# zju3dv/RelightableAvatar

Measured on AMD Instinct MI355X. Metric: rays_per_sec, higher is better.
Workload: dtype f16

## Files before the change

relightableavatar_amd/csrc/ra_hdq.hip:

```cpp
#include "ra_kernels.hpp"
#include <type_traits>
#include <cstdlib>

namespace {

constexpr int KNN_THREADS = 256;

#ifdef RA_COARSE_TS
__device__ long long ra_coarse_ts[64 * 64 * 16 * 8];
extern "C" int ra_coarse_read_timestamps(long long* out) { return (int)hipMemcpyFromSymbol(out, HIP_SYMBOL(ra_coarse_ts), sizeof(ra_coarse_ts)); }
#define RA_CSTAMP(k) do { if (tsp) { __builtin_amdgcn_sched_barrier(0); if ((threadIdx.x & 63) == 0) tsp[k] = __builtin_readcyclecounter(); __builtin_amdgcn_sched_barrier(0); } } while (0)
#else
#define RA_CSTAMP(k) do { } while (0)
#endif
constexpr int VT = 2048;

__device__ __forceinline__ void inv3d(const float R[9], float M[9]) {
    M[0] = R[4] * R[8] - R[7] * R[5];
    M[3] = -R[3] * R[8] + R[6] * R[5];
    M[6] = R[3] * R[7] - R[6] * R[4];
    M[1] = -R[1] * R[8] + R[7] * R[2];
    M[4] = R[0] * R[8] - R[6] * R[2];
    M[7] = -R[0] * R[7] + R[6] * R[1];
    M[2] = R[1] * R[5] - R[4] * R[2];
    M[5] = -R[0] * R[5] + R[3] * R[2];
    M[8] = R[0] * R[4] - R[3] * R[1];
    const float D = R[0] * M[0] + R[1] * M[3] + R[2] * M[6];
    const float inv = 1.f / (D + 1e-8f);
#pragma unroll
    for (int i = 0; i < 9; ++i) M[i] *= inv;
}

__device__ __forceinline__ float sgn(float x) { return (x > 0.f) ? 1.f : ((x < 0.f) ? -1.f : 0.f); }

__global__ void vert_blend_kernel(const float* __restrict__ weights, const float* __restrict__ A, const float* __restrict__ big_A,
                                  int n_verts, int n_bones, float* __restrict__ vertA) {
    const int v = blockIdx.x * blockDim.x + threadIdx.x;
    if (v >= n_verts) return;
    float acc[24];
#pragma unroll
    for (int e = 0; e < 24; ++e) acc[e] = 0.f;
    for (int j = 0; j < n_bones; ++j) {
        const float w = weights[(size_t)v * n_bones + j];
#pragma unroll
        for (int e = 0; e < 12; ++e) {
            acc[e] += w * A[j * 16 + e];
            acc[12 + e] += w * big_A[j * 16 + e];
        }
    }
#pragma unroll
    for (int e = 0; e < 24; ++e) vertA[(size_t)v * 24 + e] = acc[e];
}

__global__ void pack_verts_kernel(const float* __restrict__ pv, int n, float4* __restrict__ out) {
    const int v = blockIdx.x * blockDim.x + threadIdx.x;
    if (v < n) out[v] = make_float4(pv[3 * v], pv[3 * v + 1], pv[3 * v + 2], 0.f);
}

__global__ __launch_bounds__(256) void fold_bias_kernel(const float* __restrict__ W, int ld, int col0, int ncond, const float* __restrict__ cond,
                                                        const float* __restrict__ bias, float* __restrict__ out) {
    const int r = blockIdx.x * 4 + (threadIdx.x >> 6), lane = threadIdx.x & 63;
    if (r >= 256) return;
    const float* row = W + (size_t)r * ld + col0;
    float a = 0.f;
    for (int c = lane; c < ncond; c += 64) a = fmaf(row[c], cond[c], a);
#pragma unroll
    for (int o = 32; o > 0; o >>= 1) a += __shfl_xor(a, o);
    if (lane == 0) out[r] = bias[r] + a;
}

constexpr int BVH_THREADS = 1024;
constexpr int BVH_LEAF = 32;
constexpr int BVH_FAN = 8;
constexpr int BVH_MAXN = 16384;
constexpr int BVH_MAXL = BVH_MAXN / BVH_LEAF;
constexpr int BVH_MAXS = BVH_MAXL / BVH_FAN;

__device__ __forceinline__ unsigned expand10(unsigned v) {
    v = (v * 0x00010001u) & 0xFF0000FFu;
    v = (v * 0x00000101u) & 0x0F00F00Fu;
    v = (v * 0x00000011u) & 0xC30C30C3u;
    v = (v * 0x00000005u) & 0x49249249u;
    return v;
}

constexpr int RANK_WAVES = BVH_THREADS / 64;

__global__ __launch_bounds__(BVH_THREADS) void bvh_rank_kernel(const float4* __restrict__ pv, int n, int* __restrict__ order) {
    __shared__ unsigned long long keys[BVH_MAXN];
    __shared__ float red[6][BVH_THREADS / 64];
    __shared__ float bb[6];
    __shared__ int cnt[RANK_WAVES][64];
    const int tid = threadIdx.x;
    float mn[3] = {3e38f, 3e38f, 3e38f}, mx[3] = {-3e38f, -3e38f, -3e38f};
    for (int i = tid; i < n; i += BVH_THREADS) {
        const float4 v = pv[i];
        mn[0] = fminf(mn[0], v.x); mn[1] = fminf(mn[1], v.y); mn[2] = fminf(mn[2], v.z);
        mx[0] = fmaxf(mx[0], v.x); mx[1] = fmaxf(mx[1], v.y); mx[2] = fmaxf(mx[2], v.z);
    }
#pragma unroll
    for (int c = 0; c < 3; ++c)
#pragma unroll
        for (int o = 32; o > 0; o >>= 1) { mn[c] = fminf(mn[c], __shfl_xor(mn[c], o)); mx[c] = fmaxf(mx[c], __shfl_xor(mx[c], o)); }
    if ((tid & 63) == 0) for (int c = 0; c < 3; ++c) { red[c][tid >> 6] = mn[c]; red[3 + c][tid >> 6] = mx[c]; }
    __syncthreads();
    if (tid < 6) {
        float a = red[tid][0];
        for (int w = 1; w < BVH_THREADS / 64; ++w) a = tid < 3 ? fminf(a, red[tid][w]) : fmaxf(a, red[tid][w]);
        bb[tid] = a;
    }
    __syncthreads();
    const int n4 = (n + 3) & ~3;
    for (int i = tid; i < n4; i += BVH_THREADS) {
        unsigned long long k = ~0ull;
        if (i < n) {
            const float4 v = pv[i];
            const float p[3] = {v.x, v.y, v.z};
            unsigned q[3];
#pragma unroll
            for (int c = 0; c < 3; ++c) {
                const float e = fmaxf(bb[3 + c] - bb[c], 1e-12f);
                q[c] = (unsigned)fminf(fmaxf((p[c] - bb[c]) / e * 1023.f, 0.f), 1023.f);
            }
            const unsigned code = (expand10(q[0]) << 2) | (expand10(q[1]) << 1) | expand10(q[2]);
            k = ((unsigned long long)code << 32) | (unsigned)i;
        }
        keys[i] = k;
    }
    __syncthreads();
    const int lane = tid & 63, g = tid >> 6;
    const int e = blockIdx.x * 64 + lane;
    const unsigned long long mine = e < n ? keys[e] : 0ull;
    const int chunk = ((n4 / 4 + RANK_WAVES - 1) / RANK_WAVES) * 4;
    const int j0 = g * chunk, j1 = min(n4, j0 + chunk);
    int c = 0;
    for (int j = j0; j < j1; j += 4) {
        const ulonglong2 a = *reinterpret_cast<const ulonglong2*>(&keys[j]);
        const ulonglong2 b = *reinterpret_cast<const ulonglong2*>(&keys[j + 2]);
        c += (a.x < mine) + (a.y < mine) + (b.x < mine) + (b.y < mine);
    }
    cnt[g][lane] = c;
    __syncthreads();
    if (g == 0 && e < n) {
        int r = 0;
#pragma unroll
        for (int w = 0; w < RANK_WAVES; ++w) r += cnt[w][lane];
        order[r] = e;
    }
}

__global__ __launch_bounds__(BVH_THREADS) void bvh_boxes_kernel(const float4* __restrict__ pv, const int* __restrict__ order, int n,
                                                                float* __restrict__ leaves, float4* __restrict__ sbox, int nl, int ns) {
    __shared__ float lb[BVH_MAXL][6];
    const int tid = threadIdx.x, e = tid & 31;
    for (int l = tid >> 5; l < nl; l += BVH_THREADS / 32) {
        const int i = l * BVH_LEAF + e;
        float4 v = make_float4(__int_as_float(0x7f800000), __int_as_float(0x7f800000), __int_as_float(0x7f800000), __int_as_float(0x7fffffff));
        float lo[3] = {3e38f, 3e38f, 3e38f}, hi[3] = {-3e38f, -3e38f, -3e38f};
        if (i < n) {
            const int id = order[i];
            v = pv[id];
            v.w = __int_as_float(id);
            lo[0] = hi[0] = v.x; lo[1] = hi[1] = v.y; lo[2] = hi[2] = v.z;
        }
        float* soa = leaves + (size_t)l * (4 * BVH_LEAF) + e;
        soa[0] = v.x; soa[BVH_LEAF] = v.y; soa[2 * BVH_LEAF] = v.z; soa[3 * BVH_LEAF] = v.w;
#pragma unroll
        for (int c = 0; c < 3; ++c)
#pragma unroll
            for (int o = 16; o > 0; o >>= 1) { lo[c] = fminf(lo[c], __shfl_xor(lo[c], o)); hi[c] = fmaxf(hi[c], __shfl_xor(hi[c], o)); }
        if (e == 0) {
#pragma unroll
            for (int c = 0; c < 3; ++c) { lb[l][c] = lo[c]; lb[l][3 + c] = hi[c]; }
        }
    }
    __syncthreads();
    for (int sidx = tid; sidx < ns; sidx += BVH_THREADS) {
        float lo[3] = {3e38f, 3e38f, 3e38f}, hi[3] = {-3e38f, -3e38f, -3e38f};
        for (int k = 0; k < BVH_FAN; ++k) {
            const int l = sidx * BVH_FAN + k;
            if (l < nl)
#pragma unroll
                for (int c = 0; c < 3; ++c) { lo[c] = fminf(lo[c], lb[l][c]); hi[c] = fmaxf(hi[c], lb[l][3 + c]); }
        }
        sbox[2 * sidx] = make_float4(lo[0], lo[1], lo[2], 0.f);
        sbox[2 * sidx + 1] = make_float4(hi[0], hi[1], hi[2], 0.f);
        float* rec = reinterpret_cast<float*>(sbox + 2 * (size_t)ns) + (size_t)sidx * (6 * BVH_FAN);
        for (int k = 0; k < BVH_FAN; ++k) {
            const int l = sidx * BVH_FAN + k;
#pragma unroll
            for (int c = 0; c < 6; ++c) rec[12 * (k >> 1) + 2 * c + (k & 1)] = l < nl ? lb[l][c] : (c < 3 ? 3e38f : -3e38f);
        }
    }
}

template <int I, int N, typename F>
__device__ __forceinline__ void static_for(F&& f) {
    if constexpr (I < N) {
        f(std::integral_constant<int, I>{});
        static_for<I + 1, N>(f);
    }
}

template <int K>
__device__ __forceinline__ float row_bcast(float v) {
    return __int_as_float(__builtin_amdgcn_update_dpp(0, __float_as_int(v), 0x150 + K, 0xf, 0xf, false));
}

__device__ __forceinline__ float box_dist2(const float p[3], float lx, float ly, float lz, float hx, float hy, float hz) {
    const float dx = fmaxf(fmaxf(lx - p[0], p[0] - hx), 0.f);
    const float dy = fmaxf(fmaxf(ly - p[1], p[1] - hy), 0.f);
    const float dz = fmaxf(fmaxf(lz - p[2], p[2] - hz), 0.f);
    return dx * dx + dy * dy + dz * dz;
}

__device__ __forceinline__ float dist2(float dx, float dy, float dz) { return __fmaf_rn(dz, dz, __fmaf_rn(dx, dx, dy * dy)); }

__device__ __forceinline__ void knn_insert(float d, int id, float& d0, float& d1, float& d2, int& i0, int& i1, int& i2, bool dedup = false) {
    if (__builtin_expect(__ballot(d <= d2) == 0ull, 1)) return;
    bool fresh = true;
    if (dedup) fresh = (id != i0) & (id != i1) & (id != i2);
    const bool c2 = fresh && (d < d2 || (d == d2 && id < i2));
    const bool c1 = fresh && (d < d1 || (d == d1 && id < i1));
    const bool c0 = fresh && (d < d0 || (d == d0 && id < i0));
    const float nd2 = c1 ? d1 : (c2 ? d : d2);
    const int ni2 = c1 ? i1 : (c2 ? id : i2);
    const float nd1 = c0 ? d0 : (c1 ? d : d1);
    const int ni1 = c0 ? i0 : (c1 ? id : i1);
    d0 = c0 ? d : d0;
    i0 = c0 ? id : i0;
    d1 = nd1; i1 = ni1; d2 = nd2; i2 = ni2;
}

__device__ __forceinline__ void ray_point(const RaySet& rs, int i, float x[3]) {
    if (rs.mode == 0) {
        x[0] = rs.x[3 * i]; x[1] = rs.x[3 * i + 1]; x[2] = rs.x[3 * i + 2];
    } else if (rs.mode == 1) {
        const float t = rs.t[i];
        x[0] = rs.o[3 * i] + t * rs.d[3 * i];
        x[1] = rs.o[3 * i + 1] + t * rs.d[3 * i + 1];
        x[2] = rs.o[3 * i + 2] + t * rs.d[3 * i + 2];
    } else {
        const float t = rs.t[i];
        const int p = rs.pix[i], l = rs.light[i];
        x[0] = rs.o[3 * p] + t * rs.ldir[3 * l];
        x[1] = rs.o[3 * p + 1] + t * rs.ldir[3 * l + 1];
        x[2] = rs.o[3 * p + 2] + t * rs.ldir[3 * l + 2];
    }
}

template <bool BVH, int SPLIT, bool HINT = false>
__global__ __launch_bounds__(SPLIT == 1 ? KNN_THREADS : 64 * SPLIT) void hdq_coarse_kernel(FrameState fr, RaySet rs, int n_launch, float th, float inv2r2,
                                                                  HdqOut out, int dbg) {
    static_assert(SPLIT == 1 || (BVH && SPLIT >= 2 && SPLIT <= 16), "SPLIT > 1: the workgroup is SPLIT waves on the same 64 queries");
    constexpr int NT = SPLIT == 1 ? KNN_THREADS : 64 * SPLIT;
    __shared__ __attribute__((aligned(16))) unsigned char smem[BVH ? 16 : VT * 16];
#ifdef RA_COARSE_TS
    long long* tsp = blockIdx.x < 64 ? ra_coarse_ts + ((((dbg >> 8) & 63) * 64 + blockIdx.x) * 16 + (threadIdx.x >> 6)) * 8 : nullptr;
    dbg &= 255;
    if (tsp && (threadIdx.x & 63) == 0) { tsp[1] = tsp[2] = tsp[3] = tsp[4] = tsp[5] = tsp[6] = tsp[7] = 0; }
    RA_CSTAMP(0);
#endif
    const int n = rs.n_dev ? min(*rs.n_dev, n_launch) : n_launch;
    const int base = blockIdx.x * (SPLIT == 1 ? KNN_THREADS : 64);
    if (base >= n) return;
    if (blockIdx.x == 0 && threadIdx.x == 0 && out.counters) atomicAdd(&out.counters->n_coarse, (unsigned long long)n);
    const int i = base + (SPLIT == 1 ? threadIdx.x : (threadIdx.x & 63));
    const bool live_q = i < n && !(rs.skip && rs.skip[i < n ? i : 0]);
    bool live = live_q;
    if (__syncthreads_count(live_q) == 0) return;
    float x[3] = {0.f, 0.f, 0.f};
    if (live) ray_point(rs, i, x);
    const float xt[3] = {x[0] - fr.Th[0], x[1] - fr.Th[1], x[2] - fr.Th[2]};
    float p[3];
#pragma unroll
    for (int c = 0; c < 3; ++c) p[c] = xt[0] * fr.R[c] + xt[1] * fr.R[3 + c] + xt[2] * fr.R[6 + c];

    RA_CSTAMP(1);
    float d0 = 3.0e38f, d1 = 3.0e38f, d2 = 3.0e38f;
    int i0 = 0, i1 = 0, i2 = 0;
    if (dbg & 1) { d0 = 1e-4f; d1 = 2e-4f; d2 = 3e-4f; i0 = 0; i1 = 1; i2 = 2; }
    else if (BVH) {
        const int nl = fr.bvh_leaves, ns = fr.bvh_supers;
        if (!live) { d0 = d1 = d2 = -1.f; }
        const unsigned long long lm = __ballot(live);
        const int first = lm ? __ffsll((long long)lm) - 1 : 0;
        const int lane = threadIdx.x & 63;
        typedef float f2 __attribute__((ext_vector_type(2)));
        const f2 px2 = {p[0], p[0]}, py2 = {p[1], p[1]}, pz2 = {p[2], p[2]};
        constexpr bool hinted = HINT;
#ifdef RA_COARSE_TS
        int n_rare = 0;
#endif
        typedef float f8 __attribute__((ext_vector_type(8)));
        typedef float f4 __attribute__((ext_vector_type(4)));
        typedef int i4 __attribute__((ext_vector_type(4)));
        auto soa8 = [&](int off) __attribute__((always_inline)) { return *(const f8 __attribute__((address_space(4)))*)(fr.bvh_soa + off); };
        auto soa_id4 = [&](int off) __attribute__((always_inline)) { return *(const i4 __attribute__((address_space(4)))*)(fr.bvh_soa + off); };
        auto box4 = [&](int off) __attribute__((always_inline)) {
            return *(const f4 __attribute__((address_space(4)))*)(reinterpret_cast<const float*>(fr.bvh_sbox) + off);
        };
        auto box1 = [&](int off) __attribute__((always_inline)) { return reinterpret_cast<const float*>(fr.bvh_sbox)[off]; };
        auto scan_leaf = [&](int l) __attribute__((always_inline)) {
            const int L = l * (4 * BVH_LEAF);
            f8 cx = soa8(L), cy = soa8(L + BVH_LEAF), cz = soa8(L + 2 * BVH_LEAF), nx = cx, ny = cy, nz = cz;
            static_for<0, 4>([&](auto q_) {
                constexpr int q = decltype(q_)::value;
                static_for<0, 2>([&](auto g_) {
                    constexpr int g = decltype(g_)::value;
                    const f2 ax = {cx[4 * g], cx[4 * g + 1]}, ay = {cy[4 * g], cy[4 * g + 1]}, az = {cz[4 * g], cz[4 * g + 1]};
                    const f2 bx = {cx[4 * g + 2], cx[4 * g + 3]}, by = {cy[4 * g + 2], cy[4 * g + 3]}, bz = {cz[4 * g + 2], cz[4 * g + 3]};
                    const f2 dxa = px2 - ax, dya = py2 - ay, dza = pz2 - az, dxb = px2 - bx, dyb = py2 - by, dzb = pz2 - bz;
                    f2 da = dya * dya, db = dyb * dyb;
                    da = __builtin_elementwise_fma(dxa, dxa, da);
                    db = __builtin_elementwise_fma(dxb, dxb, db);
                    da = __builtin_elementwise_fma(dza, dza, da);
                    db = __builtin_elementwise_fma(dzb, dzb, db);
                    if (__builtin_expect(__ballot(fminf(fminf(da.x, da.y), fminf(db.x, db.y)) <= d2) != 0ull, 0)) {
#ifdef RA_COARSE_TS
                        ++n_rare;
#endif
                        const i4 id = soa_id4(L + 3 * BVH_LEAF + 8 * q + 4 * g);
                        knn_insert(da.x, id.x, d0, d1, d2, i0, i1, i2, hinted);
                        knn_insert(da.y, id.y, d0, d1, d2, i0, i1, i2, hinted);
                        knn_insert(db.x, id.z, d0, d1, d2, i0, i1, i2, hinted);
                        knn_insert(db.y, id.w, d0, d1, d2, i0, i1, i2, hinted);
                    }
                    if constexpr (g == 0 && q < 3) { nx = soa8(L + 8 * (q + 1)); ny = soa8(L + BVH_LEAF + 8 * (q + 1)); nz = soa8(L + 2 * BVH_LEAF + 8 * (q + 1)); }
                });
                cx = nx; cy = ny; cz = nz;
            });
        };
        int n_scan = 0, n_open = 0;
        if (lm != 0ull) {
            int seed = -1;
            if (hinted) {
                if (live) {
                    float e[3]; int h[3];
#pragma unroll
                    for (int k = 0; k < 3; ++k) {
                        h[k] = rs.hint_src ? rs.hint_src[3 * (size_t)rs.hint_src_index[i] + k] : rs.nn_hint[3 * (size_t)i + k];
                        const float4 v = fr.pverts4[h[k]];
                        e[k] = dist2(p[0] - v.x, p[1] - v.y, p[2] - v.z);
                    }
                    auto before = [&](int a, int b) { return e[a] < e[b] || (e[a] == e[b] && h[a] < h[b]); };
                    auto swap = [&](int a, int b) { const float te = e[a]; e[a] = e[b]; e[b] = te; const int th_ = h[a]; h[a] = h[b]; h[b] = th_; };
                    if (before(1, 0)) swap(0, 1);
                    if (before(2, 1)) swap(1, 2);
                    if (before(1, 0)) swap(0, 1);
                    d0 = e[0]; d1 = e[1]; d2 = e[2]; i0 = h[0]; i1 = h[1]; i2 = h[2];
                }
            } else {
                auto bc = [&](float v) __attribute__((always_inline)) { return __int_as_float(__builtin_amdgcn_readlane(__float_as_int(v), first)); };
                const float q[3] = {bc(p[0]), bc(p[1]), bc(p[2])};
                auto wave_argmin = [&](float d) __attribute__((always_inline)) {
                    float m = d;
#pragma unroll
                    for (int o = 32; o > 0; o >>= 1) m = fminf(m, __shfl_xor(m, o));
                    return __ffsll((long long)__ballot(d == m)) - 1;
                };
                float d = 3.4e38f;
                if (lane < ns) { const int o = 8 * lane; d = box_dist2(q, box1(o), box1(o + 1), box1(o + 2), box1(o + 4), box1(o + 5), box1(o + 6)); }
                const int bi = wave_argmin(d);
                d = 3.4e38f;
                if (lane < BVH_FAN) { const int o = 8 * ns + bi * (6 * BVH_FAN) + 12 * (lane >> 1) + (lane & 1); d = box_dist2(q, box1(o), box1(o + 2), box1(o + 4), box1(o + 6), box1(o + 8), box1(o + 10)); }
                seed = bi * BVH_FAN + wave_argmin(d);
            }
            RA_CSTAMP(2);
            if (!hinted) {
                n_scan = 1;
                scan_leaf(seed);
            }
            RA_CSTAMP(3);
#pragma unroll 1
            for (int j = SPLIT > 1 ? (int)(threadIdx.x >> 6) : 0; j < ns; j += SPLIT) {
                const f4 slo = box4(8 * j), shi = box4(8 * j + 4);
                if (__ballot(box_dist2(p, slo.x, slo.y, slo.z, shi.x, shi.y, shi.z) * 0.99999f <= d2) == 0ull) continue;
                ++n_open;
#pragma unroll 1
                for (int pr = 0; pr < BVH_FAN / 2; ++pr) {
                    const int ro = 8 * ns + j * (6 * BVH_FAN) + 12 * pr;
                    const f4 ra = box4(ro), rb = box4(ro + 4), rc = box4(ro + 8);
                    const f2 ax = f2{ra.x, ra.y} - px2, ay = f2{ra.z, ra.w} - py2, az = f2{rb.x, rb.y} - pz2;
                    const f2 bx = px2 - f2{rb.z, rb.w}, by = py2 - f2{rc.x, rc.y}, bz = pz2 - f2{rc.z, rc.w};
                    const f2 ex = {__builtin_fmaxf(__builtin_fmaxf(ax.x, bx.x), 0.f), __builtin_fmaxf(__builtin_fmaxf(ax.y, bx.y), 0.f)};
                    const f2 ey = {__builtin_fmaxf(__builtin_fmaxf(ay.x, by.x), 0.f), __builtin_fmaxf(__builtin_fmaxf(ay.y, by.y), 0.f)};
                    const f2 ez = {__builtin_fmaxf(__builtin_fmaxf(az.x, bz.x), 0.f), __builtin_fmaxf(__builtin_fmaxf(az.y, bz.y), 0.f)};
                    f2 dd = ex * ex;
                    dd = __builtin_elementwise_fma(ey, ey, dd);
                    dd = __builtin_elementwise_fma(ez, ez, dd);
                    dd *= 0.99999f;
                    const int l = j * BVH_FAN + 2 * pr;
                    if (l != seed && __ballot(dd.x <= d2) != 0ull) { scan_leaf(l); ++n_scan; }
                    if (l + 1 != seed && __ballot(dd.y <= d2) != 0ull) { scan_leaf(l + 1); ++n_scan; }
                }
            }
        }
        RA_CSTAMP(4);
#ifdef RA_COARSE_TS
        if (tsp && (threadIdx.x & 63) == 0) tsp[7] = ((long long)n_scan << 32) | ((long long)n_rare << 12) | n_open;
#endif
        if (SPLIT > 1) {
            __shared__ float md[SPLIT > 1 ? SPLIT - 1 : 1][3][64];
            __shared__ int mi[SPLIT > 1 ? SPLIT - 1 : 1][3][64];
            const int wv = threadIdx.x >> 6;
            if (wv > 0) {
                md[wv - 1][0][lane] = d0; md[wv - 1][1][lane] = d1; md[wv - 1][2][lane] = d2;
                mi[wv - 1][0][lane] = i0; mi[wv - 1][1][lane] = i1; mi[wv - 1][2][lane] = i2;
            }
            __syncthreads();
            if (wv == 0) {
#pragma unroll
                for (int w = 0; w < SPLIT - 1; ++w)
#pragma unroll
                    for (int k = 0; k < 3; ++k) {
                        const int id = mi[w][k][lane];
                        const bool dup = id == i0 || id == i1 || id == i2;
                        knn_insert(dup ? 3.4e38f : md[w][k][lane], id, d0, d1, d2, i0, i1, i2);
                    }
            } else {
                live = false;
            }
        }
        RA_CSTAMP(5);
        if ((dbg & 4) && out.counters && lane == 0) {
            atomicAdd(&out.counters->n_shadow_rays, (unsigned long long)n_scan);
            atomicAdd(&out.counters->n_hit_pixels, (unsigned long long)n_open);
        }
    } else {
        float4* sv = reinterpret_cast<float4*>(smem);
        for (int v0 = 0; v0 < fr.n_verts; v0 += VT) {
            const int nv = min(VT, fr.n_verts - v0);
            __syncthreads();
            for (int j = threadIdx.x; j < nv; j += KNN_THREADS) sv[j] = fr.pverts4[v0 + j];
            __syncthreads();
#pragma unroll 4
            for (int j = 0; j < nv; ++j) {
                const float4 v = sv[j];
                const float dx = p[0] - v.x, dy = p[1] - v.y, dz = p[2] - v.z;
                const float d = dist2(dx, dy, dz);
                knn_insert(d, v0 + j, d0, d1, d2, i0, i1, i2);
            }
        }
    }
    if (rs.nn_hint && live) {
        int* hw = rs.nn_hint + 3 * (size_t)i;
        hw[0] = i0; hw[1] = i1; hw[2] = i2;
    }
    if (dbg & 2) { if (live) out.sdf[i] = d0 + d1 + d2 + (float)(i0 + i1 + i2); return; }
    float dk[3] = {d0, d1, d2};
    int ik[3] = {i0, i1, i2};
    float sk[3];
#pragma unroll
    for (int k = 0; k < 3; ++k) {
        const float4 v = fr.pverts4[ik[k]];
        const float* nn = fr.pnorm + 3 * (size_t)ik[k];
        const float dot = (p[0] - v.x) * nn[0] + (p[1] - v.y) * nn[1] + (p[2] - v.z) * nn[2];
        sk[k] = sqrtf(dk[k]) * sgn(dot);
    }
    const float th2 = th * th;
    if (!(dbg & 32)) {
        const float* t0 = fr.tverts + 3 * (size_t)ik[0];
#pragma unroll
        for (int k = 1; k < 3; ++k) {
            const float* tk = fr.tverts + 3 * (size_t)ik[k];
            const float ex = tk[0] - t0[0], ey = tk[1] - t0[1], ez = tk[2] - t0[2];
            if (!(ex * ex + ey * ey + ez * ez < th2)) { dk[k] = dk[0]; ik[k] = ik[0]; sk[k] = sk[0]; }
        }
    }
    float smpl = (sk[0] + sk[1] + sk[2]) / 3.f;
    if (dbg & 32) {
        const float sg = fmaxf(fmaxf(sgn(sk[0]), sgn(sk[1])), sgn(sk[2]));
        smpl = sqrtf((dk[0] + dk[1] + dk[2]) / 3.f) * sg;
        sk[0] = sk[1] = sk[2] = smpl;
    }
    smpl = (smpl < -th) ? smpl : fabsf(smpl);
    const bool fine = live && (d0 < th2);
    if (live) {
        out.sdf[i] = smpl;
        if (out.raw_zero && !fine) {
            float* rz = out.raw_zero + (size_t)i * out.raw_C;
            for (int c = 0; c < out.raw_C; ++c) rz[c] = 0.f;
        }
        if (out.dbg_sdf_batch) {
#pragma unroll
            for (int k = 0; k < 3; ++k) { out.dbg_sdf_batch[3 * i + k] = sk[k]; out.dbg_nn_batch[3 * i + k] = ik[k]; out.dbg_d2[3 * i + k] = dk[k]; }
        }
    }
    __shared__ int wcount[NT / 64 + 1], wcount2[NT / 64 + 1];
    const bool fine2 = fine && out.key != nullptr && out.key[rs.light[i]] != 0;
    const unsigned long long m = __ballot(fine && !fine2), m2 = out.key ? __ballot(fine2) : 0ull;
    const int lane = threadIdx.x & 63, wv = threadIdx.x >> 6;
    if (lane == 0) { wcount[wv] = __popcll(m); wcount2[wv] = __popcll(m2); }
    __syncthreads();
    if (threadIdx.x == 0) {
        int tot = 0, tot2 = 0;
#pragma unroll
        for (int w = 0; w < NT / 64; ++w) { const int cnt = wcount[w]; wcount[w] = tot; tot += cnt; const int c2 = wcount2[w]; wcount2[w] = tot2; tot2 += c2; }
        wcount[NT / 64] = (dbg & 8) ? base : (tot ? atomicAdd(out.fine_count, tot) : 0);
        wcount2[NT / 64] = tot2 ? atomicAdd(out.fine_count2, tot2) : 0;
    }
    __syncthreads();
    RA_CSTAMP(6);
    if (!fine || (dbg & 16)) return;
    const int slot = fine2 ? wcount2[NT / 64] + wcount2[wv] + __popcll(m2 & ((1ull << lane) - 1ull))
                           : wcount[NT / 64] + wcount[wv] + __popcll(m & ((1ull << lane) - 1ull));
    float w[3], ws = 0.f;
#pragma unroll
    for (int k = 0; k < 3; ++k) { w[k] = expf(-dk[k] * inv2r2); ws += w[k]; }
    ws += 1.1920928955078125e-07f;
    float M[24];
#pragma unroll
    for (int e = 0; e < 24; ++e) M[e] = 0.f;
#pragma unroll
    for (int k = 0; k < 3; ++k) {
        const float wk = w[k] / ws;
        const float4* src = reinterpret_cast<const float4*>(fr.vertA + (size_t)ik[k] * 24);
#pragma unroll
        for (int q = 0; q < 6; ++q) {
            const float4 a = src[q];
            M[4 * q] += wk * a.x; M[4 * q + 1] += wk * a.y; M[4 * q + 2] += wk * a.z; M[4 * q + 3] += wk * a.w;
        }
    }
    const float AR[9] = {M[0], M[1], M[2], M[4], M[5], M[6], M[8], M[9], M[10]};
    float Ai[9];
    inv3d(AR, Ai);
    const float q[3] = {p[0] - M[3], p[1] - M[7], p[2] - M[11]};
    float tp[3], bp[3];
#pragma unroll
    for (int r = 0; r < 3; ++r) tp[r] = Ai[3 * r] * q[0] + Ai[3 * r + 1] * q[1] + Ai[3 * r + 2] * q[2];
#pragma unroll
    for (int r = 0; r < 3; ++r) bp[r] = M[12 + 4 * r] * tp[0] + M[12 + 4 * r + 1] * tp[1] + M[12 + 4 * r + 2] * tp[2] + M[12 + 4 * r + 3];
    if (fine2) {
        out.fine_idx2[slot] = i;
        out.bpts2[3 * slot] = bp[0]; out.bpts2[3 * slot + 1] = bp[1]; out.bpts2[3 * slot + 2] = bp[2];
        return;
    }
    out.fine_idx[slot] = i;
    out.bpts[3 * slot] = bp[0]; out.bpts[3 * slot + 1] = bp[1]; out.bpts[3 * slot + 2] = bp[2];
    if (out.mats) {
        float4* dst = reinterpret_cast<float4*>(out.mats + (size_t)slot * 24);
#pragma unroll
        for (int qd = 0; qd < 6; ++qd) dst[qd] = make_float4(M[4 * qd], M[4 * qd + 1], M[4 * qd + 2], M[4 * qd + 3]);
    }
    if (out.dbg_bpts) {
#pragma unroll
        for (int c = 0; c < 3; ++c) { out.dbg_bpts[3 * i + c] = bp[c]; out.dbg_tpts[3 * i + c] = tp[c]; }
#pragma unroll
        for (int e = 0; e < 24; ++e) out.dbg_mats[(size_t)i * 24 + e] = M[e];
    }
}

}

void launch_vert_blend(const float* weights, const float* A, const float* big_A, int n_verts, int n_bones, float* vertA,
                       hipStream_t s) {
    hipLaunchKernelGGL(vert_blend_kernel, dim3((n_verts + 255) / 256), dim3(256), 0, s, weights, A, big_A, n_verts, n_bones, vertA);
}

void launch_pack_verts(const float* pverts, int n_verts, float4* out, hipStream_t s) {
    hipLaunchKernelGGL(pack_verts_kernel, dim3((n_verts + 255) / 256), dim3(256), 0, s, pverts, n_verts, out);
}

void launch_fold_bias(const float* W, int ld, int col0, int ncond, const float* cond, const float* bias, float* out,
                      hipStream_t s) {
    hipLaunchKernelGGL(fold_bias_kernel, dim3(64), dim3(256), 0, s, W, ld, col0, ncond, cond, bias, out);
}

int bvh_leaf_count(int n_verts) {
    if (n_verts > BVH_MAXN) return 0;
    return (n_verts + BVH_LEAF - 1) / BVH_LEAF;
}
int bvh_super_count(int n_leaves) { return (n_leaves + BVH_FAN - 1) / BVH_FAN; }

void launch_bvh_build(const float4* pverts4, int n_verts, int* order, float* leaves, float4* sbox, int n_leaves, int n_supers, hipStream_t s) {
    hipLaunchKernelGGL(bvh_rank_kernel, dim3((n_verts + 63) / 64), dim3(BVH_THREADS), 0, s, pverts4, n_verts, order);
    hipLaunchKernelGGL(bvh_boxes_kernel, dim3(1), dim3(BVH_THREADS), 0, s, pverts4, order, n_verts, leaves, sbox, n_leaves, n_supers);
}

void launch_hdq_coarse(const FrameState& fr, const RaySet& rs, int n, float th, float blend_radius, const HdqOut& out,
                       hipStream_t s, bool geodesic) {
    if (n <= 0) return;
    const float inv2r2 = 1.f / (2.f * blend_radius * blend_radius);
    const dim3 grid((n + KNN_THREADS - 1) / KNN_THREADS);
    int dbg = 0, probe = 0, split_max = 196608;
#ifdef RA_TESTING
    static const int e_dbg = getenv("RA_COARSE_DBG") ? atoi(getenv("RA_COARSE_DBG")) : 0;
    static const int e_probe = getenv("RA_COARSE_PROBE") ? atoi(getenv("RA_COARSE_PROBE")) : 0;
    static const int e_split = getenv("RA_COARSE_SPLIT_MAX") ? atoi(getenv("RA_COARSE_SPLIT_MAX")) : 196608;
    dbg = e_dbg; probe = e_probe; split_max = e_split;
#endif
    if (!geodesic) dbg |= 32;
#ifdef RA_COARSE_TS
    static int launch_no = 0;
    dbg |= (launch_no++ & 63) << 8;
#endif
    const bool hint = (rs.nn_hint != nullptr && rs.hint_valid != 0) || rs.hint_src != nullptr;
    for (int pass = probe ? 0 : 1; pass < 2; ++pass) {
        const int d = pass == 0 ? probe : dbg;
        if (fr.bvh_leaves > 0 && n <= split_max)
        {
            const int groups = (n + 63) / 64;
            if (hint) {
                if (n <= split_max / 8) hipLaunchKernelGGL((hdq_coarse_kernel<true, 16, true>), dim3(groups), dim3(1024), 0, s, fr, rs, n, th, inv2r2, out, d);
                else if (n <= split_max / 2) hipLaunchKernelGGL((hdq_coarse_kernel<true, 8, true>), dim3(groups), dim3(512), 0, s, fr, rs, n, th, inv2r2, out, d);
                else hipLaunchKernelGGL((hdq_coarse_kernel<true, 4, true>), dim3(groups), dim3(256), 0, s, fr, rs, n, th, inv2r2, out, d);
            } else {
                if (n <= split_max / 8) hipLaunchKernelGGL((hdq_coarse_kernel<true, 16>), dim3(groups), dim3(1024), 0, s, fr, rs, n, th, inv2r2, out, d);
                else if (n <= split_max / 2) hipLaunchKernelGGL((hdq_coarse_kernel<true, 8>), dim3(groups), dim3(512), 0, s, fr, rs, n, th, inv2r2, out, d);
                else hipLaunchKernelGGL((hdq_coarse_kernel<true, 4>), dim3(groups), dim3(256), 0, s, fr, rs, n, th, inv2r2, out, d);
            }
        }
        else if (fr.bvh_leaves > 0 && hint) hipLaunchKernelGGL((hdq_coarse_kernel<true, 1, true>), grid, dim3(KNN_THREADS), 0, s, fr, rs, n, th, inv2r2, out, d);
        else if (fr.bvh_leaves > 0) hipLaunchKernelGGL((hdq_coarse_kernel<true, 1>), grid, dim3(KNN_THREADS), 0, s, fr, rs, n, th, inv2r2, out, d);
        else hipLaunchKernelGGL((hdq_coarse_kernel<false, 1>), grid, dim3(KNN_THREADS), 0, s, fr, rs, n, th, inv2r2, out, d);
        if (pass == 0) hipMemsetAsync(out.fine_count, 0, sizeof(int), s);
    }
}
```

Baseline: 9.053 million.

## Prefilter hinted BVH super boxes by wave bounding box and skip duplicate inserts

```diff
diff --git a/relightableavatar_amd/csrc/ra_hdq.hip b/relightableavatar_amd/csrc/ra_hdq.hip
--- a/relightableavatar_amd/csrc/ra_hdq.hip
+++ b/relightableavatar_amd/csrc/ra_hdq.hip
@@ -7,7 +7,8 @@
 constexpr int KNN_THREADS = 256;
 
 #ifdef RA_COARSE_TS
-__device__ long long ra_coarse_ts[64 * 64 * 16 * 8];
+constexpr int RA_TS_WORDS = 12;
+__device__ long long ra_coarse_ts[64 * 64 * 16 * RA_TS_WORDS];
 extern "C" int ra_coarse_read_timestamps(long long* out) { return (int)hipMemcpyFromSymbol(out, HIP_SYMBOL(ra_coarse_ts), sizeof(ra_coarse_ts)); }
 #define RA_CSTAMP(k) do { if (tsp) { __builtin_amdgcn_sched_barrier(0); if ((threadIdx.x & 63) == 0) tsp[k] = __builtin_readcyclecounter(); __builtin_amdgcn_sched_barrier(0); } } while (0)
 #else
@@ -214,12 +215,31 @@
     return dx * dx + dy * dy + dz * dz;
 }
 
+__device__ __forceinline__ float box_dist2_range(const float pl[3], const float ph[3], float lx, float ly, float lz, float hx, float hy, float hz) {
+    const float dx = fmaxf(fmaxf(lx - ph[0], pl[0] - hx), 0.f);
+    const float dy = fmaxf(fmaxf(ly - ph[1], pl[1] - hy), 0.f);
+    const float dz = fmaxf(fmaxf(lz - ph[2], pl[2] - hz), 0.f);
+    return dx * dx + dy * dy + dz * dz;
+}
+
+template <bool MAX>
+__device__ __forceinline__ int wave_minmax(int v) {
+    auto op = [](int a, int b) __attribute__((always_inline)) { return MAX ? max(a, b) : min(a, b); };
+    v = op(v, __builtin_amdgcn_update_dpp(0, v, 0xB1, 0xf, 0xf, true));
+    v = op(v, __builtin_amdgcn_update_dpp(0, v, 0x4E, 0xf, 0xf, true));
+    v = op(v, __builtin_amdgcn_update_dpp(0, v, 0x141, 0xf, 0xf, true));
+    v = op(v, __builtin_amdgcn_update_dpp(0, v, 0x140, 0xf, 0xf, true));
+    return op(op(__builtin_amdgcn_readlane(v, 0), __builtin_amdgcn_readlane(v, 16)), op(__builtin_amdgcn_readlane(v, 32), __builtin_amdgcn_readlane(v, 48)));
+}
+__device__ __forceinline__ int float_key(int b) { return b ^ ((b >> 31) & 0x7fffffff); }
+
 __device__ __forceinline__ float dist2(float dx, float dy, float dz) { return __fmaf_rn(dz, dz, __fmaf_rn(dx, dx, dy * dy)); }
 
-__device__ __forceinline__ void knn_insert(float d, int id, float& d0, float& d1, float& d2, int& i0, int& i1, int& i2, bool dedup = false) {
-    if (__builtin_expect(__ballot(d <= d2) == 0ull, 1)) return;
+__device__ __forceinline__ void knn_insert(float d, int id, float& d0, float& d1, float& d2, int& i0, int& i1, int& i2, bool dedup = false,
+                                           bool fresh_guard = false) {
     bool fresh = true;
     if (dedup) fresh = (id != i0) & (id != i1) & (id != i2);
+    if (__builtin_expect(__ballot(d <= d2 && (fresh || !fresh_guard)) == 0ull, 1)) return;
     const bool c2 = fresh && (d < d2 || (d == d2 && id < i2));
     const bool c1 = fresh && (d < d1 || (d == d1 && id < i1));
     const bool c0 = fresh && (d < d0 || (d == d0 && id < i0));
@@ -256,9 +276,9 @@
     constexpr int NT = SPLIT == 1 ? KNN_THREADS : 64 * SPLIT;
     __shared__ __attribute__((aligned(16))) unsigned char smem[BVH ? 16 : VT * 16];
 #ifdef RA_COARSE_TS
-    long long* tsp = blockIdx.x < 64 ? ra_coarse_ts + ((((dbg >> 8) & 63) * 64 + blockIdx.x) * 16 + (threadIdx.x >> 6)) * 8 : nullptr;
+    long long* tsp = blockIdx.x < 64 ? ra_coarse_ts + ((((dbg >> 8) & 63) * 64 + blockIdx.x) * 16 + (threadIdx.x >> 6)) * RA_TS_WORDS : nullptr;
     dbg &= 255;
-    if (tsp && (threadIdx.x & 63) == 0) { tsp[1] = tsp[2] = tsp[3] = tsp[4] = tsp[5] = tsp[6] = tsp[7] = 0; }
+    if (tsp && (threadIdx.x & 63) == 0) { for (int k = 1; k < RA_TS_WORDS; ++k) tsp[k] = 0; }
     RA_CSTAMP(0);
 #endif
     const int n = rs.n_dev ? min(*rs.n_dev, n_launch) : n_launch;
@@ -289,8 +309,13 @@
         typedef float f2 __attribute__((ext_vector_type(2)));
         const f2 px2 = {p[0], p[0]}, py2 = {p[1], p[1]}, pz2 = {p[2], p[2]};
         constexpr bool hinted = HINT;
-#ifdef RA_COARSE_TS
-        int n_rare = 0;
+#ifdef RA_TESTING
+        const bool prefilter = !(dbg & 64), fresh_guard = !(dbg & 128);
+#else
+        constexpr bool prefilter = true, fresh_guard = true;
+#endif
+#ifdef RA_COARSE_TS
+        int n_rare = 0, n_dup = 0, n_tested = 0, n_pair = 0, n_pair_fail = 0;
 #endif
         typedef float f8 __attribute__((ext_vector_type(8)));
         typedef float f4 __attribute__((ext_vector_type(4)));
@@ -317,14 +342,18 @@
                     da = __builtin_elementwise_fma(dza, dza, da);
                     db = __builtin_elementwise_fma(dzb, dzb, db);
                     if (__builtin_expect(__ballot(fminf(fminf(da.x, da.y), fminf(db.x, db.y)) <= d2) != 0ull, 0)) {
+                        const i4 id = soa_id4(L + 3 * BVH_LEAF + 8 * q + 4 * g);
 #ifdef RA_COARSE_TS
                         ++n_rare;
-#endif
-                        const i4 id = soa_id4(L + 3 * BVH_LEAF + 8 * q + 4 * g);
-                        knn_insert(da.x, id.x, d0, d1, d2, i0, i1, i2, hinted);
-                        knn_insert(da.y, id.y, d0, d1, d2, i0, i1, i2, hinted);
-                        knn_insert(db.x, id.z, d0, d1, d2, i0, i1, i2, hinted);
-                        knn_insert(db.y, id.w, d0, d1, d2, i0, i1, i2, hinted);
+                        if (hinted) {
+                            auto passes = [&](float d, int v) { return d <= d2 && v != i0 && v != i1 && v != i2; };
+                            n_dup += __ballot(passes(da.x, id.x) || passes(da.y, id.y) || passes(db.x, id.z) || passes(db.y, id.w)) == 0ull;
+                        }
+#endif
+                        knn_insert(da.x, id.x, d0, d1, d2, i0, i1, i2, hinted, hinted && fresh_guard);
+                        knn_insert(da.y, id.y, d0, d1, d2, i0, i1, i2, hinted, hinted && fresh_guard);
+                        knn_insert(db.x, id.z, d0, d1, d2, i0, i1, i2, hinted, hinted && fresh_guard);
+                        knn_insert(db.y, id.w, d0, d1, d2, i0, i1, i2, hinted, hinted && fresh_guard);
                     }
                     if constexpr (g == 0 && q < 3) { nx = soa8(L + 8 * (q + 1)); ny = soa8(L + BVH_LEAF + 8 * (q + 1)); nz = soa8(L + 2 * BVH_LEAF + 8 * (q + 1)); }
                 });
@@ -372,10 +401,12 @@
                 scan_leaf(seed);
             }
             RA_CSTAMP(3);
-#pragma unroll 1
-            for (int j = SPLIT > 1 ? (int)(threadIdx.x >> 6) : 0; j < ns; j += SPLIT) {
+            auto sweep_box = [&](int j) __attribute__((always_inline)) {
                 const f4 slo = box4(8 * j), shi = box4(8 * j + 4);
-                if (__ballot(box_dist2(p, slo.x, slo.y, slo.z, shi.x, shi.y, shi.z) * 0.99999f <= d2) == 0ull) continue;
+#ifdef RA_COARSE_TS
+                ++n_tested;
+#endif
+                if (__ballot(box_dist2(p, slo.x, slo.y, slo.z, shi.x, shi.y, shi.z) * 0.99999f <= d2) == 0ull) return;
                 ++n_open;
 #pragma unroll 1
                 for (int pr = 0; pr < BVH_FAN / 2; ++pr) {
@@ -391,14 +422,54 @@
                     dd = __builtin_elementwise_fma(ez, ez, dd);
                     dd *= 0.99999f;
                     const int l = j * BVH_FAN + 2 * pr;
+#ifdef RA_COARSE_TS
+                    const int n_scan_before = n_scan;
+#endif
                     if (l != seed && __ballot(dd.x <= d2) != 0ull) { scan_leaf(l); ++n_scan; }
                     if (l + 1 != seed && __ballot(dd.y <= d2) != 0ull) { scan_leaf(l + 1); ++n_scan; }
+#ifdef RA_COARSE_TS
+                    ++n_pair;
+                    n_pair_fail += n_scan == n_scan_before;
+#endif
                 }
+            };
+            if constexpr (hinted) {
+                static_assert(BVH_MAXS <= 64, "one candidate bit per super box");
+                unsigned long long cand = ns >= 64 ? ~0ull : (1ull << ns) - 1ull;
+                if constexpr (SPLIT > 1) cand &= (~0ull / ((1ull << SPLIT) - 1ull)) << __builtin_amdgcn_readfirstlane((int)(threadIdx.x >> 6));
+                if (prefilter) {
+                    float wl[3], wh[3];
+#pragma unroll
+                    for (int c = 0; c < 3; ++c) {
+                        const int k = float_key(__float_as_int(p[c]));
+                        const bool in = live && p[c] == p[c];
+                        wl[c] = __int_as_float(float_key(wave_minmax<false>(in ? k : 0x7fffffff)));
+                        wh[c] = __int_as_float(float_key(wave_minmax<true>(in ? k : (int)0x80000000)));
+                    }
+                    const float rmax = __int_as_float(wave_minmax<true>(d2 == d2 ? __float_as_int(d2) : __float_as_int(-1.f)));
+                    bool may = false;
+                    if (lane < ns) {
+                        const float4 lo = fr.bvh_sbox[2 * lane], hi = fr.bvh_sbox[2 * lane + 1];
+                        may = box_dist2_range(wl, wh, lo.x, lo.y, lo.z, hi.x, hi.y, hi.z) * 0.99999f <= rmax;
+                    }
+                    cand &= __ballot(may);
+                }
+                while (cand != 0ull) {
+                    const int j = __ffsll((long long)cand) - 1;
+                    cand &= cand - 1ull;
+                    sweep_box(j);
+                }
+            } else {
+#pragma unroll 1
+                for (int j = SPLIT > 1 ? (int)(threadIdx.x >> 6) : 0; j < ns; j += SPLIT) sweep_box(j);
             }
         }
         RA_CSTAMP(4);
 #ifdef RA_COARSE_TS
-        if (tsp && (threadIdx.x & 63) == 0) tsp[7] = ((long long)n_scan << 32) | ((long long)n_rare << 12) | n_open;
+        if (tsp && (threadIdx.x & 63) == 0) {
+            tsp[7] = ((long long)n_scan << 32) | ((long long)n_rare << 12) | n_open;
+            tsp[8] = n_tested; tsp[9] = n_dup; tsp[10] = n_pair; tsp[11] = n_pair_fail;
+        }
 #endif
         if (SPLIT > 1) {
             __shared__ float md[SPLIT > 1 ? SPLIT - 1 : 1][3][64];
@@ -588,7 +659,8 @@
     static const int e_dbg = getenv("RA_COARSE_DBG") ? atoi(getenv("RA_COARSE_DBG")) : 0;
     static const int e_probe = getenv("RA_COARSE_PROBE") ? atoi(getenv("RA_COARSE_PROBE")) : 0;
     static const int e_split = getenv("RA_COARSE_SPLIT_MAX") ? atoi(getenv("RA_COARSE_SPLIT_MAX")) : 196608;
-    dbg = e_dbg; probe = e_probe; split_max = e_split;
+    auto off = [](const char* name) { const char* v = getenv(name); return v && atoi(v) == 0; };
+    dbg = e_dbg | (off("RA_COARSE_PREFILTER") ? 64 : 0) | (off("RA_COARSE_FRESH_GUARD") ? 128 : 0); probe = e_probe; split_max = e_split;
 #endif
     if (!geodesic) dbg |= 32;
 #ifdef RA_COARSE_TS
```

After: 9.024 million. Within noise of the previous version (-0.3%).
